# neverorfrog/vehicle-control

Hardware: AMD Instinct MI355X
Metric: MPC solves/sec (batched, N=20) (higher is better)
Workload: dtype f64; 1 GPU; C2 kinematic-bicycle LTV-MPC, B=1024 per GPU, N=20, fp64; batch_per_gpu=1024, global_batch=1024, horizon=20, parallelism=dp1 (independent shards)

## Files before the change

### include/vcmpc.h

```cpp
#ifndef VCMPC_H
#define VCMPC_H

#include <stdint.h>

#ifdef __cplusplus
extern "C" {
#endif

#define VCMPC_ABI_VERSION 13
#define VC_MAX_OBSTACLES 16

typedef struct vc_ctx vc_ctx;

enum vc_model { VC_MODEL_KINEMATIC = 0, VC_MODEL_DYNAMIC = 1, VC_MODEL_CASCADED = 2 };
enum vc_dtype { VC_F64 = 0, VC_F32 = 1 };
enum vc_flags { VC_HOST_PTRS = 0, VC_DEVICE_PTRS = 1 };
enum vc_tyre { VC_TYRE_FIALA = 0, VC_TYRE_LINEAR = 1 };
enum vc_status { VC_SOLVED = 0, VC_MAX_ITER = 1, VC_NONFINITE = 2, VC_OUT_OF_DOMAIN = 3, VC_INFEASIBLE = 4 };
enum vc_error {
  VC_OK = 0,
  VC_E_ARG = -1,
  VC_E_HIP = -2,
  VC_E_UNSUPPORTED = -3
};
// ... 71 lines not shown
int vc_abi_version(void);
int vc_params_sizeof(void);

vc_ctx* vc_create(int device, int model, int N, int max_batch, int dtype, const vc_params* params);
void vc_destroy(vc_ctx* ctx);
const char* vc_last_error(const vc_ctx* ctx);

int vc_set_stream(vc_ctx* ctx, void* stream);

int vc_set_obstacles(vc_ctx* ctx, int n, const double* s, const double* ey, const double* radius,
                     double margin_min);
int vc_synchronize(vc_ctx* ctx);

int vc_set_infeasibility(vc_ctx* ctx, int on, double eps);

int vc_get_farkas(vc_ctx* ctx, int B, void* y, int flags);

int vc_set_sqp_infeasibility(vc_ctx* ctx, int on, double eps);

int vc_get_sqp_farkas(vc_ctx* ctx, int B, void* y, int32_t* qp_index, int flags);

int vc_set_sqp_regularization(vc_ctx* ctx, int levels, double factor);

int vc_get_sqp_regularization(vc_ctx* ctx, int B, int32_t* level, int flags);

int vc_set_casc_infeasibility(vc_ctx* ctx, int on, double eps);

int vc_get_casc_farkas(vc_ctx* ctx, int B, void* y, int32_t* qp_index, int flags);

int vc_solve(vc_ctx* ctx, int B, const void* x0, const void* kappa, const void* ds,
             void* xbar, void* ubar, void* u0, int32_t* status, int32_t* iters, int flags);

int vc_solve_from(vc_ctx* ctx, int B, const void* x0, const void* kappa, const void* ds, const void* ubar_in,
                  void* xbar, void* u_out, void* u0, int32_t* status, int32_t* iters, int flags);

int vc_solve_diag(vc_ctx* ctx, int B, const void* x0, const void* kappa, const void* ds,
                  void* xbar, void* ubar, void* u0, int32_t* status, int32_t* iters, void* diag,
                  int flags);

int vc_solve_debug(vc_ctx* ctx, int B, const void* x0, const void* kappa, const void* ds, void* xbar, void* ubar,
                   void* u0, int32_t* status, int32_t* iters, void* dbg, int flags);
int vc_debug_stride(void);

int vc_debug_qp_fault(vc_ctx* ctx, int sqp_iter, int problem);

int vc_debug_kin_merit(vc_ctx* ctx, int B, const void* x0, const void* kappa, const void* ds, const void* u_prev,
                       void* u, const void* x_prev, void* x, int32_t* status, int32_t* iters, int32_t* st_acc,
                       int32_t* it_acc, int first, int restart, void* u0, void* ls_diag, int flags);

int vc_debug_sqp_breakdown(vc_ctx* ctx, int sqp_iter, int problem, int levels);

int vc_debug_rcp(vc_ctx* ctx, int n, const void* x, void* out, int flags);

int vc_rollout(vc_ctx* ctx, int B, const void* x0, const void* ubar, const void* kappa,
               const void* ds, void* xbar, int flags);

int vc_linearize(vc_ctx* ctx, int B, const void* xbar, const void* ubar, const void* kappa,
                 const void* ds, void* A, void* Bm, int flags);

int vc_condense(vc_ctx* ctx, int B, const void* x0, const void* ubar, const void* kappa,
                const void* ds, void* H, void* g, int flags);

int vc_plant_step(vc_ctx* ctx, int B, const void* x, const void* u, const void* kappa,
                  double dt, void* x_next, int flags);

int vc_spatial_step(vc_ctx* ctx, int B, const void* x, const void* u, const void* kappa,
                    const void* ds, void* x_next, int flags);

int vc_ode(vc_ctx* ctx, int B, const void* x, const void* u, const void* kappa, int space, void* f, int flags);

int vc_track_set(vc_ctx* ctx, int n_pieces, double h, double length, const double* coef);

int vc_track_k(vc_ctx* ctx, int B, const void* s, void* k, int flags);

int vc_horizon(vc_ctx* ctx, int B, const void* x0, const void* xbar, double mpc_dt, void* kappa, void* ds,
               int flags);

int vc_drive(vc_ctx* ctx, int B, double* x64, const void* u0, double dt, void* x_ctx, int flags);

int vc_simulate(vc_ctx* ctx, int B, int steps, double mpc_dt, double dt, double* x64, void* xbar, void* ubar,
                double* log_x, void* log_u, int32_t* nfail, int flags);

#ifdef __cplusplus
}
#endif
#endif
```

### vehicle-control_amd/csrc/kin_ltv.hip

```cpp
#include <hip/hip_runtime.h>

#include <cstdint>

#include "vc_kernels.hpp"
#include "vc_models.hpp"
#include "vcmpc.h"

#ifndef KIN_NU_TOL
#define KIN_NU_TOL 1e-10
#endif
#ifndef KIN_EARLY_F
#define KIN_EARLY_F 100.0
#endif
#ifndef KIN_EARLY_ROUNDS
#define KIN_EARLY_ROUNDS 2
#endif
#ifndef KIN_TAPIA_F
#define KIN_TAPIA_F 1.02
#endif
#ifndef KIN_DUAL_TOL
#define KIN_DUAL_TOL 1e-12
#endif
#ifndef KIN_AL_RHO
#define KIN_AL_RHO 1e1
// ... 136 lines not shown
  alignas(16) double zrow[48];
  double xb[N + 1][KIN_NX + 1];
  double jac[N + 1][9];
  double ub[D::n];
  double kap[N], ds[N];
  union {
    struct {
      double vz[64];
      double vc[64];
    };
    alignas(16) double tb2[128];
  };
  double dinv[64];
#if KIN_XPOSE_ONCE
  alignas(16) double tb3[8 * 18];
#endif
};
static_assert(sizeof(Smem<20>) <= 40960, "LDS of one problem: four must fit a CU's 160 KB");

template <int N>
__host__ __device__ constexpr int crow_stage(int r) {
  return r < N - 1 ? r + 1 : r - (N - 1) + 1;
}

template <int LEN, int SA, int SB, int CH = KIN_DOT_CH>
__device__ __forceinline__ double lds_dot(lds_cdouble* a, lds_cdouble* b) {
  constexpr int NCH = (LEN + CH - 1) / CH;
  double ca[2][CH], cb[2][CH];
  auto fetch = [&](int c, int buf) {
#pragma unroll
    for (int q = 0; q < CH; ++q) {
      const int i = c * CH + q;
      ca[buf][q] = (i < LEN) ? a[i * SA] : 0.0;
      cb[buf][q] = (i < LEN) ? b[i * SB] : 0.0;
    }
  };
  double a0 = 0.0, a1 = 0.0;
  fetch(0, 0);
#pragma unroll
  for (int c = 0; c < NCH; ++c) {
    if (c + 1 < NCH) fetch(c + 1, (c + 1) & 1);
    fence();
#pragma unroll
    for (int q = 0; q < CH; q += 2) {
      a0 += ca[c & 1][q] * cb[c & 1][q];
      a1 += ca[c & 1][q + 1] * cb[c & 1][q + 1];
    }
  }
  fence();
  return a0 + a1;
}

template <int N>
__device__ double grow_dot(const Smem<N>& s, int lane) {
  constexpr int NC = Dims<N>::NC;
  const int r = lane < NC ? lane : 0;
  const double a = lds_dot<2 * (N - 1), 1, 1>(lds_opaque(&s.G[r][0]), lds_opaque(&s.vz[0]));
  return lane < NC ? a : 0.0;
}

template <int N>
__device__ double gt_dot(const Smem<N>& s, int lane) {
  constexpr int n = Dims<N>::n, NC = Dims<N>::NC, LD = Dims<N>::LD;
  const int j = lane < n ? lane : 0;
  const double a = lds_dot<NC, LD, 1>(lds_opaque(&s.G[0][j]), lds_opaque(&s.vc[0]));
  return lane < n ? a : 0.0;
}


template <int N>
__device__ double h_dot(const Smem<N>& s, int lane) {
  constexpr int n = Dims<N>::n;
  const int j = lane < n ? lane : 0;
  return lds_dot<n, 1, 1>(lds_opaque(&s.H[j][0]), lds_opaque(&s.vz[0]));
}

__device__ __forceinline__ void kin_sincos(double x, double& sn, double& cs) {
  const double n = __builtin_rint(x * 6.36619772367581382433e-01);
  const double y = fma(-n, 6.07710050650619224932e-11, fma(-n, 1.57079632673412561417e+00, x));
  const double z = y * y;
  const double rs = fma(z, fma(z, fma(z, fma(z, 1.58969099521155010221e-10, -2.50507602534068634195e-08),
                                      2.75573137070700676789e-06), -1.98412698298579493134e-04),
                        8.33333333332248946124e-03);
  const double sk = fma(z * y, fma(z, rs, -1.66666666666666324348e-01), y);
  const double rc = z * fma(z, fma(z, fma(z, fma(z, fma(z, -1.13596475577881948265e-11, 2.08757232129817482790e-09),
                                                  -2.75573143513906633035e-07), 2.48015872894767294178e-05),
                                   -1.38888888888741095749e-03), 4.16666666666666019037e-02);
  const double hz = 0.5 * z, w = 1.0 - hz;
  const double ck = w + (((1.0 - w) - hz) + z * rc);
  const int q = int(n) & 3;
  const double a = (q & 1) ? ck : sk, b = (q & 1) ? sk : ck;
  sn = (q & 2) ? -a : a;
  cs = ((q + 1) & 2) ? -b : b;
}

__device__ __forceinline__ double rsq_nr(double d) {
  double inv = __builtin_amdgcn_rsq(d);
#if KIN_RSQ_HALLEY
  const double e = fma(-d, inv * inv, 1.0);
  return fma(inv * e, fma(0.375, e, 0.5), inv);
#else
  inv = inv * (1.5 - 0.5 * d * inv * inv);
  inv = inv * (1.5 - 0.5 * d * inv * inv);
  return inv;
#endif
}

template <int N>
__device__ __forceinline__ void store_rows(const double (&Mr)[Dims<N>::n], Smem<N>& s, int lane) {
}

template <int N>
struct RowRegs {
  int lo[Dims<N>::n], hi[Dims<N>::n];
};
template <int N>
__device__ __forceinline__ void row_put(RowRegs<N>& R, int k, double v) {
  asm("v_accvgpr_write_b32 %0, %1" : "=a"(R.lo[k]) : "v"(__double2loint(v)));
  asm("v_accvgpr_write_b32 %0, %1" : "=a"(R.hi[k]) : "v"(__double2hiint(v)));
// ... 682 lines not shown
    bx.hasLo = bx.hasHi = (lane < n);
    const int st = crow_stage<N>(lane < NC ? lane : 0);
    if (lane < N - 1) {
      cs.lo = W.v_min - s.xb[st][0];
      cs.hi = 0.0;
      cs.hasLo = true; cs.hasHi = false;
    } else if (lane < NC) {
      cs.lo = W.delta_min - s.xb[st][1];
      cs.hi = W.delta_max - s.xb[st][1];
      cs.hasLo = cs.hasHi = true;
    } else {
      cs.lo = cs.hi = 0.0;
      cs.hasLo = cs.hasHi = false;
    }
  }
  const double mtot = double(4 * N + 3 * (N - 1));
  double scale, hdiag_max;
  {
    double m = fabs(gj);
    if (bx.hasLo) m = fmax(m, fabs(bx.lo));
    if (bx.hasHi) m = fmax(m, fabs(bx.hi));
    if (cs.hasLo) m = fmax(m, fabs(cs.lo));
    if (cs.hasHi) m = fmax(m, fabs(cs.hi));
    scale = 1.0 + wave_max(m);
    hdiag_max = fmax(wave_max(hjj), 1.0);
  }
  double z = 0.0;
  bx.slo = bx.hasLo ? fmax(-bx.lo, 1.0) : 1.0;
  bx.shi = bx.hasHi ? fmax(bx.hi, 1.0) : 1.0;
  bx.llo = bx.hasLo ? 1.0 : 0.0;
  bx.lhi = bx.hasHi ? 1.0 : 0.0;
  cs.slo = cs.hasLo ? fmax(-cs.lo, 1.0) : 1.0;
  cs.shi = cs.hasHi ? fmax(cs.hi, 1.0) : 1.0;
  cs.llo = cs.hasLo ? 1.0 : 0.0;
  cs.lhi = cs.hasHi ? 1.0 : 0.0;

  VC_TACC(T_SETUP, t_setup0)
  const int max_iter = A.qp.max_iter;
  const double tol = A.qp.tol * scale;
  int it = 0;
  bool converged = false, chol_fail = false, near = false;
  double last_res = 0.0, last_mu = 0.0;
  RowRegs<N> Mr;
  double rd = 0.0, rlo_b = 0.0, rhi_b = 0.0, rlo_c = 0.0, rhi_c = 0.0;
  auto true_residuals = [&]() {
    wave_sync();
    s.vz[lane] = (lane < n) ? z : 0.0;
    s.vc[lane] = (lane < NC) ? (cs.lhi - cs.llo) : 0.0;
    wave_sync();
    const double yc = grow_dot<N>(s, lane);
    fence();
    const double hz = h_dot<N>(s, lane);
    fence();
    rd = (lane < n) ? (hz + gj + (bx.lhi - bx.llo) + gt_dot<N>(s, lane)) : 0.0;
    rlo_b = bx.hasLo ? (z - bx.lo - bx.slo) : 0.0;
    rhi_b = bx.hasHi ? (bx.hi - z - bx.shi) : 0.0;
    rlo_c = cs.hasLo ? (yc - cs.lo - cs.slo) : 0.0;
    rhi_c = cs.hasHi ? (cs.hi - yc - cs.shi) : 0.0;
  };
  auto max_residual = [&]() {
    return wave_max(fmax(fmax(fabs(rd), fmax(fabs(rlo_b), fabs(rhi_b))), fmax(fabs(rlo_c), fabs(rhi_c))));
  };
  int tapb = 0;
  const double tol_early = KIN_EARLY_F > 0.0 ? fmax(tol, KIN_EARLY_F * tol) : tol;
  int e_set = 0;
#ifdef VC_TIMING
  uint64_t e_fmask = 0;
  bool e_row = false, e_have = false;
#endif
  double tol_cur = tol_early;
  bool polished = false, pchol_fail = false;
  int rounds = 0;
#pragma unroll 1
  for (;;) {
  if (finite) {
#pragma unroll 1
    for (;;) {
      no_hoist();
      VC_TSTAMP(t_res0)
      if (it == 0) true_residuals();
      const double mu = wave_sum(__builtin_fma(cs.shi, cs.lhi,
                                               __builtin_fma(cs.slo, cs.llo,
                                                             __builtin_fma(bx.shi, bx.lhi, bx.slo * bx.llo)))) / mtot;
      double res = max_residual();
      if (it > 0 && res <= tol_cur && mu <= tol_cur) {
        true_residuals();
        res = max_residual();
      }
      converged = res <= tol_cur && mu <= tol_cur;
      last_res = res;
      last_mu = mu;
      if (converged || it >= max_iter || !isfinite(res) || !isfinite(mu)) break;
      ++it;
      const double wlo_b = bx.hasLo ? bx.llo / bx.slo : 0.0;
      const double whi_b = bx.hasHi ? bx.lhi / bx.shi : 0.0;
      const double wlo_c = cs.hasLo ? cs.llo / cs.slo : 0.0;
      const double whi_c = cs.hasHi ? cs.lhi / cs.shi : 0.0;
      wave_sync();
      s.vc[lane] = (lane < NC) ? wlo_c + whi_c : 0.0;
      wave_sync();
      VC_TACC(T_RESID, t_res0)
      VC_TSTAMP(t_build0)
      d4 nacc[Tiles<N>::NT];
      build_normal_acc<N>(nacc, s, wlo_b + whi_b, hjj, lane);
      VC_TACC(T_BUILD, t_build0)
      VC_TSTAMP(t_chol0)
      const bool chol_ok = factor_blocked<N>(Mr, nacc, s, lane);
      VC_TACC(T_CHOL, t_chol0)
      if (!chol_ok) {
        chol_fail = true;
        near = res <= 1e-6 * scale && mu <= tol;
        break;
      }
#ifdef VC_TIMING
      const uint64_t t_sol_before = tacc[T_SOLVE];
#endif
      VC_TSTAMP(t_step0)
      const double islo_b = bx.hasLo ? rcp_nr(bx.slo) : 0.0, ishi_b = bx.hasHi ? rcp_nr(bx.shi) : 0.0;
      const double islo_c = cs.hasLo ? rcp_nr(cs.slo) : 0.0, ishi_c = cs.hasHi ? rcp_nr(cs.shi) : 0.0;
      const double illo_b = bx.hasLo ? rcp_nr(bx.llo) : 0.0, ilhi_b = bx.hasHi ? rcp_nr(bx.lhi) : 0.0;
      const double illo_c = cs.hasLo ? rcp_nr(cs.llo) : 0.0, ilhi_c = cs.hasHi ? rcp_nr(cs.lhi) : 0.0;
      double sm = 0.0, pp1 = 0.0, pp2 = 0.0, pp3 = 0.0, pp4 = 0.0;
#pragma unroll 1
      for (int pass = 0; pass < 2; ++pass) {
        no_hoist();
        const double rclo_b = __builtin_fma(bx.slo, bx.llo, pp1) - sm, rchi_b = __builtin_fma(bx.shi, bx.lhi, pp2) - sm;
        const double rclo_c = __builtin_fma(cs.slo, cs.llo, pp3) - sm, rchi_c = __builtin_fma(cs.shi, cs.lhi, pp4) - sm;
        const double thi_b = ishi_b * -rchi_b, thi_c = ishi_c * -rchi_c;
        const double tlo_b = islo_b * rclo_b, tlo_c = islo_c * rclo_c;
        const double eb = (bx.hasHi ? __builtin_fma(-whi_b, rhi_b, thi_b) : 0.0) +
                          (bx.hasLo ? __builtin_fma(wlo_b, rlo_b, tlo_b) : 0.0);
        const double ec = (cs.hasHi ? __builtin_fma(-whi_c, rhi_c, thi_c) : 0.0) +
                          (cs.hasLo ? __builtin_fma(wlo_c, rlo_c, tlo_c) : 0.0);
        wave_sync();
        s.vc[lane] = (lane < NC) ? ec : 0.0;
        wave_sync();
        const double rhs = (lane < n) ? (-rd - eb - gt_dot<N>(s, lane)) : 0.0;
        VC_TSTAMP(t_sol0)
        const double dz = chol_solve<N>(Mr, s, rhs, lane);
        VC_TACC(T_SOLVE, t_sol0)
        wave_sync();
        s.vz[lane] = (lane < n) ? dz : 0.0;
        wave_sync();
        const double dyc = grow_dot<N>(s, lane);
        const double d1 = bx.hasLo ? dz + rlo_b : 0.0;
        const double d2 = bx.hasLo ? __builtin_fma(islo_b, -rclo_b, -(wlo_b * (dz + rlo_b))) : 0.0;
        const double d3 = bx.hasHi ? rhi_b - dz : 0.0;
        const double d4 = bx.hasHi ? __builtin_fma(-whi_b, rhi_b - dz, thi_b) : 0.0;
        const double e1 = cs.hasLo ? dyc + rlo_c : 0.0;
        const double e2 = cs.hasLo ? __builtin_fma(islo_c, -rclo_c, -(wlo_c * (dyc + rlo_c))) : 0.0;
        const double e3 = cs.hasHi ? rhi_c - dyc : 0.0;
        const double e4 = cs.hasHi ? __builtin_fma(-whi_c, rhi_c - dyc, thi_c) : 0.0;
        const double tmax = wave_max(fmax(fmax(fmax(-d1 * islo_b, -d2 * illo_b), fmax(-d3 * ishi_b, -d4 * ilhi_b)),
                                          fmax(fmax(-e1 * islo_c, -e2 * illo_c), fmax(-e3 * ishi_c, -e4 * ilhi_c))));
        const double amax = 1.0 / fmax(1.0, tmax);
        if (pass == 0) {
          const double mua = wave_sum((bx.slo + amax * d1) * (bx.llo + amax * d2) +
                                      (bx.shi + amax * d3) * (bx.lhi + amax * d4) +
                                      (cs.slo + amax * e1) * (cs.llo + amax * e2) +
                                      (cs.shi + amax * e3) * (cs.lhi + amax * e4)) / mtot;
          const double sr = mua / mu;
          sm = sr * sr * sr * mu;
          pp1 = d1 * d2; pp2 = d3 * d4; pp3 = e1 * e2; pp4 = e3 * e4;
        } else {
          const double al = KIN_STEP_F * amax;
          {
            auto tap = [&](double dl, double il, double dsv, double is) -> int {
              const double lr = fma(al * dl, il, 1.0), sr = fma(al * dsv, is, 1.0);
              return lr > KIN_TAPIA_F * sr ? 1 : (sr > KIN_TAPIA_F * lr ? 2 : 0);
            };
            tapb = tap(d2, illo_b, d1, islo_b) | (tap(d4, ilhi_b, d3, ishi_b) << 2) |
                   (tap(e2, illo_c, e1, islo_c) << 4) | (tap(e4, ilhi_c, e3, ishi_c) << 6);
          }
          z = (lane < n) ? z + al * dz : z;
          bx.slo += al * d1; bx.llo += al * d2; bx.shi += al * d3; bx.lhi += al * d4;
          cs.slo += al * e1; cs.llo += al * e2; cs.shi += al * e3; cs.lhi += al * e4;
          const double om = 1.0 - al;
          rd *= om; rlo_b *= om; rhi_b *= om; rlo_c *= om; rhi_c *= om;
        }
      }
      VC_TACC(T_STEP, t_step0)
#ifdef VC_TIMING
      tacc[T_STEP] -= tacc[T_SOLVE] - t_sol_before;
#endif
    }
  }

  VC_TSTAMP(t_pol0)
  if ((converged || near) && A.qp.polish > 0) {
    constexpr double AL_RHO = KIN_AL_RHO;
// ... 47 lines not shown
      const double rho_new = (act && gn2 > 1e-28) ? AL_RHO * hdiag_max / gn2 : 0.0;
      const double rho_c = (KIN_UPDATE && rho_k > 0.0 && rho_new > 0.0) ? rho_k : rho_new;
      const double bnd_c = act ? ((alo_c ? cs.lo : cs.hi) - gfix) : 0.0;
      const double base = (lane < n) ? -(gj + h_dot<N>(s, lane)) : 0.0;
      wave_sync();
      s.vc[lane] = rho_c;
      wave_sync();
      VC_TSTAMP(t_pf0)
      bool updated = false;
      if (KIN_UPDATE && upd != 0) {
        const bool same = __ballot(lane < NC && rho_c != rho_k && !(upd == 2 && lane == upd_j)) == 0ull;
        VC_TSTAMP(t_u0)
        if (same) updated = factor_update<N>(Mr, s, upd, upd_j, fixed, sqrt(lane_bcast(rho_c, upd_j)), lane);
#ifdef VC_TIMING
        if (updated) tacc[T_NUPD] += 1;
#endif
        VC_TACC(T_UCYC, t_u0)
      }
      rho_k = rho_c;
      if (!updated) {
        d4 pacc[Tiles<N>::NT];
        build_normal_acc<N>(pacc, s, 0.0, hjj, lane);
        const int pl = lane_opaque(lane), plr = pl >> 4, plc = pl & 15;
#pragma unroll
        for (int I = 0, t = 0; I < Tiles<N>::NB; ++I) {
#pragma unroll
          for (int J = 0; J <= I; ++J, ++t) {
            const int c = 16 * J + plc;
            const bool fc = (fmask >> c) & 1ull;
#pragma unroll
            for (int q = 0; q < 4; ++q) {
              const int r = 16 * I + plr + 4 * q;
              const bool fr = (fmask >> r) & 1ull;
              pacc[t][q] = (fr || fc) ? (r == c ? 1.0 : 0.0) : pacc[t][q];
            }
          }
        }
        if (!factor_blocked<N>(Mr, pacc, s, lane)) {
          pchol_fail = true;
          break;
        }
      }
      VC_TACC(T_UPDATE, t_pf0)
      VC_TSTAMP(t_pal0)
      double nu_c = (act && rho_c > 0.0) ? ((ahi_c ? cs.lhi : 0.0) - (alo_c ? cs.llo : 0.0)) : 0.0;

      const bool al_act = act && rho_c > 0.0;
      const double bnd_al = alo_c ? cs.lo : cs.hi;
      double zp = 0.0, emax = 0.0;
      {
        wave_sync();
        s.vc[lane] = (lane < NC) ? (nu_c - rho_c * bnd_c) : 0.0;
        wave_sync();
        const double rhs = (lane < n) ? (fixed ? zfix : (base - gt_dot<N>(s, lane))) : 0.0;
        zp = chol_solve<N>(Mr, s, rhs, lane);
        wave_sync();
        s.vz[lane] = (lane < n) ? zp : 0.0;
        wave_sync();
        const double yr = grow_dot<N>(s, lane);
        double rr = al_act ? (yr - bnd_al) : 0.0;
        const double ie = 1.0 / (1e-14 * scale), inu = KIN_NU_TOL > 0.0 ? 1.0 / (KIN_NU_TOL * scale) : 0.0;
        auto crit = [&](double r) { return wave_max(fmax(fabs(r) * ie, fabs(rho_c * r) * inu)); };
#ifdef VC_TIMING
        tacc[T_PPASS] += 1;
#endif
        if (crit(rr) > 1.0) {
          double pd = rho_c * rr;
          double rz = wave_sum(rr * pd);
#pragma unroll 1
          for (int it = 1; it < AL_MAX; ++it) {
            no_hoist();
            wave_sync();
            s.vc[lane] = (lane < NC) ? pd : 0.0;
            wave_sync();
            const double gtp = gt_dot<N>(s, lane);
            const double zq = chol_solve<N>(Mr, s, (lane < n && !fixed) ? gtp : 0.0, lane);
            wave_sync();
            s.vz[lane] = (lane < n) ? zq : 0.0;
            wave_sync();
            const double gq = grow_dot<N>(s, lane);
            const double q = al_act ? gq : 0.0;
            const double pq = wave_sum(pd * q);
#ifdef VC_TIMING
            tacc[T_PPASS] += 1;
#endif
            if (!(pq > 0.0)) break;
            const double al = rz / pq;
            nu_c = fma(al, pd, nu_c);
            zp = fma(-al, zq, zp);
            rr = fma(-al, q, rr);
            if (crit(rr) <= 1.0) break;
            const double zt = rho_c * rr;
            const double rzn = wave_sum(rr * zt);
            pd = fma(rzn / rz, pd, zt);
            rz = rzn;
          }
        }
      }
      VC_TACC(T_PAL, t_pal0)
      wave_sync();
      s.vz[lane] = (lane < n) ? zp : 0.0;
      s.vc[lane] = (lane < NC) ? nu_c : 0.0;
      wave_sync();
      const double grad = (lane < n) ? (h_dot<N>(s, lane) + gj + gt_dot<N>(s, lane)) : 0.0;
      const double ypc = grow_dot<N>(s, lane);
#if KIN_STAT_CHECK
      emax = wave_max(fmax(al_act ? fabs(ypc - bnd_al) : 0.0, (lane < n && !fixed) ? fabs(grad) : 0.0));
#else
      emax = wave_max(al_act ? fabs(ypc - bnd_al) : 0.0);
#endif
      const double dv_b = (lane < n) ? (ahi_b ? grad : (alo_b ? -grad : -1.0)) : -1.0;
      const double dv_c = (lane < NC) ? (ahi_c ? -nu_c : (alo_c ? nu_c : -1.0)) : -1.0;
      const double pv_b = (lane < n && !fixed) ? fmax(bx.lo - zp, zp - bx.hi) : -1.0;
      const double pv_c = (lane < NC && !(act && rho_c > 0.0))
                              ? fmax(cs.hasLo ? cs.lo - ypc : -1.0, cs.hasHi ? ypc - cs.hi : -1.0)
                              : -1.0;
      const double dmax = wave_max(fmax(dv_b, dv_c));
      const double pmax = wave_max(fmax(pv_b, pv_c));
      if (dmax <= dtol && pmax <= ptol) {
        if (emax <= ptol) {
          z = (lane < n) ? zp : z;
          polished = true;
        }
        break;
      }
      const bool dual = dmax > dtol;
      const double worst = dual ? dmax : pmax;
      const double vb = dual ? dv_b : pv_b, vcr = dual ? dv_c : pv_c;
      const uint64_t who = __ballot(fmax(vb, vcr) == worst);
      const int sel = __builtin_ffsll((long long)who) - 1;
      const bool sel_box = (__ballot(vb >= vcr) >> sel) & 1ull;
      upd = dual ? 0 : (sel_box ? 1 : 2);
      upd_j = sel;
#ifdef VC_TIMING
      if (dual) tacc[T_NDROP] += 1;
#endif
      if (lane == sel) {
        if (vb >= vcr) {
          if (dual) { alo_b = false; ahi_b = false; }
          else if (zp < bx.lo) alo_b = true;
          else ahi_b = true;
        } else {
          if (dual) { alo_c = false; ahi_c = false; }
          else if (ypc < cs.lo) alo_c = true;
          else ahi_c = true;
        }
      }
#ifdef VC_TIMING
      int r0code = 0;
      if (tol_cur > tol && round == 0) {
        int tside = 0;
        if (vb >= vcr) tside = (dual ? (ahi_b ? (tapb >> 2) : tapb) : (zp < bx.lo ? tapb : (tapb >> 2))) & 3;
        else tside = (dual ? (ahi_c ? (tapb >> 6) : (tapb >> 4)) : (ypc < cs.lo ? (tapb >> 4) : (tapb >> 6))) & 3;
        const int code = 1 + (dual ? 2 : (vb >= vcr ? 0 : 1)) + 3 * tside;
        r0code = __builtin_amdgcn_readlane(code, sel);
#ifdef VC_TIMING
        tacc[T_R0CHG] = (uint64_t)r0code;
// ... 48 lines not shown
  }
  {
    const double y = grow_dot<N>(s, lane);
    const int slot = lane < N - 1 ? 64 + lane + 1
                                  : (lane < NC ? n + (lane - (N - 1)) + 1 : (lane == NC ? 64 : (lane == NC + 1 ? n : 127)));
    wave_sync();
    s.tb2[slot] = y;
    wave_sync();
    double ey = 0.0, ep = 0.0, eyk = 0.0, epk = 0.0;
#pragma unroll 4
    for (int k = 0; k < N; ++k) {
      const double h = s.ds[k], dd = s.vz[n + k];
      eyk = lane_put(eyk, ey, k);
      epk = lane_put(epk, ep, k);
      const double ney = ey + h * (s.jac[k][4] * ey + s.jac[k][5] * ep);
      const double nep = ep + h * (s.jac[k][6] * dd + s.jac[k][7] * ey + s.jac[k][8] * ep);
      ey = ney; ep = nep;
    }
    eyk = lane_put(eyk, ey, N);
    epk = lane_put(epk, ep, N);
    const double eyn = __shfl_down(eyk, 1), epn = __shfl_down(epk, 1);
    const int k = lane < N ? lane : 0;
    const double q = s.jac[k][0], qv = s.jac[k][1], qey = s.jac[k][2], qep = s.jac[k][3];
    const double h = s.ds[k], a = s.ub[2 * k], w = s.ub[2 * k + 1];
    const double da = s.vz[2 * k], dw = s.vz[2 * k + 1];
    const double dv = s.vc[k], dd = s.vz[n + k];
    const double dq = qv * dv + qey * eyk + qep * epk;
    const double dt = wave_prefix(lane < N ? h * dq : 0.0, lane);
    wave_sync();
    if (lane < N) {
      double* xr = s.xb[k + 1];
      xr[0] += dv + h * (a * dq + q * da);
      xr[1] += dd + h * (w * dq + q * dw);
      xr[3] += eyn;
      xr[4] += epn;
      xr[5] += dt;
    }
    wave_sync();
    double* xo = A.x_out + (size_t)b * (N + 1) * KIN_NX;
    for (int i = lane; i < (N + 1) * KIN_NX; i += 64) xo[i] = s.xb[i / KIN_NX][i % KIN_NX];
  }
  VC_TACC(T_OUT, t_out0)
  VC_TACC(T_TOTAL, t_all0)
#ifdef VC_TIMING
  if (A.diag && lane < T_NSLOT) {
    double v = 0.0;
#pragma unroll
    for (int i = 0; i < T_NSLOT; ++i) v = (i == lane) ? double(tacc[i]) : v;
    A.diag[(size_t)b * (4 + T_NSLOT) + 4 + lane] = v;
  }
#endif
}

size_t kin_ltv_smem_bytes(int N) {
  switch (N) {
    case 20: return sizeof(Smem<20>);
    default: return 0;
  }
}

hipError_t launch_kin_ltv(const KinLtvArgs& a, int N, hipStream_t stream) {
  if (a.B <= 0) return hipSuccess;
  switch (N) {
    case 20:
      hipLaunchKernelGGL(kin_ltv_kernel<20>, dim3(a.B), dim3(64), 0, stream, a);
      return hipGetLastError();
    default:
      return hipErrorInvalidValue;
  }
}

}
```

### vehicle-control_amd/csrc/vc_kernels.hpp

```cpp
#pragma once
#include <hip/hip_runtime.h>

#include <cstddef>
#include <cstdint>

#include "vc_models.hpp"
#include "vcmpc.h"

#ifdef VC_TIMING
#define VC_DIAG_COLS 16
#define VC_DYN_DIAG_COLS 19
#define VC_CASC_DIAG_COLS 17
#define VC_ST_DIAG_COLS 13
#else
#define VC_DIAG_COLS 4
#define VC_DYN_DIAG_COLS 4
#define VC_CASC_DIAG_COLS 4
#define VC_ST_DIAG_COLS 4
#endif

#define VC_OBS_MARGIN_MIN 0.05

namespace vc {

// ... 198 lines not shown
  double* u0;
  int32_t* status;
  int32_t* iters;
  double* diag;
  double* jws;
  double* H_out;
  double* g_out;
  int mode;
  int B;
  DynCoef<double> car;
  vc_dyn_mpc w;
  vc_casc_mpc cw;
  vc_qp qp;
  vc_obstacles obs;
  int detect;
  double detect_eps;
  double* farkas;
  int32_t* qp_index;
};

struct ModelArgs {
  int model;
  int B, N;
  int M;
  int shift;
  double L;
  DynCoef<double> dyn64;
  DynCoef<float> dyn32;
};
template <typename T>
__host__ __device__ inline const DynCoef<T>& dyn_coef(const ModelArgs& m);
template <>
__host__ __device__ inline const DynCoef<double>& dyn_coef<double>(const ModelArgs& m) { return m.dyn64; }
template <>
__host__ __device__ inline const DynCoef<float>& dyn_coef<float>(const ModelArgs& m) { return m.dyn32; }

struct TrackTable {
  const double* coef;
  int n;
  double h, length;
};

hipError_t launch_track_k(const TrackTable& tt, int dtype, int B, const void* s, void* k, hipStream_t st);
hipError_t launch_horizon(const TrackTable& tt, int model, int dtype, int B, int N, int M, double ds_pm,
                          const void* x0, bool x0_fp64, const void* xbar, double mpc_dt, void* kappa, void* ds,
                          void* x0_out, hipStream_t st);
hipError_t launch_drive(const ModelArgs& m, int dtype, const TrackTable& tt, double* x64, const void* u0, double dt,
                        void* x_ctx, const int32_t* status, void* xbar, void* ubar, int32_t* nfail, double* log_x,
                        void* log_u, const void* kappa, hipStream_t st);
hipError_t launch_kin_ltv(const KinLtvArgs& a, int N, hipStream_t stream);
hipError_t launch_kin_ric(const KinLtvArgs& a, int N, hipStream_t stream);
hipError_t launch_kin_merit(const KinMeritArgs& a, hipStream_t stream);
hipError_t launch_rcp_probe(int n, const double* x, double* out, hipStream_t st);
hipError_t launch_kin_qp_fault(const KinLtvArgs& a, int N, int b, hipStream_t stream);
bool kin_ric_built(int N);
hipError_t launch_dyn_sqp(const DynSqpArgs& a, int N, hipStream_t stream);
hipError_t launch_casc_sqp(const CascSqpArgs& a, int N, int M, hipStream_t stream);
hipError_t launch_casc_ric(const CascSqpArgs& a, int N, int M, hipStream_t stream);
bool casc_ric_built(int N, int M);
size_t casc_ric_jws_doubles(int N, int M, int B);
hipError_t launch_st_sqp(const StSqpArgs& a, int N, hipStream_t stream);
hipError_t launch_st_sqp_reg(const StSqpArgs& a, int N, hipStream_t stream);
bool st_sqp_built(int N);
size_t st_sqp_jws_doubles(int N, int B);
bool casc_sqp_built(int N, int M);
size_t dyn_sqp_smem_bytes(int N);
int dyn_sqp_debug_stride();
size_t kin_ltv_smem_bytes(int N);
hipError_t launch_ode(const ModelArgs& m, int dtype, const void* x, const void* u, const void* kappa, int space,
                      void* f, hipStream_t st);
hipError_t launch_plant_step(const ModelArgs& m, int dtype, const void* x, const void* u, const void* kappa, double dt,
                             void* xn, hipStream_t st);
hipError_t launch_spatial_step(const ModelArgs& m, int dtype, const void* x, const void* u, const void* kappa,
                               const void* ds, void* xn, hipStream_t st);
hipError_t launch_rollout(const ModelArgs& m, int dtype, const void* x0, const void* ubar, const void* kappa,
                          const void* ds, void* xbar, hipStream_t st);
hipError_t launch_kin_linearize(const ModelArgs& m, const void* xbar, const void* ubar, const void* kappa,
                                const void* ds, void* A, void* Bm, hipStream_t st);

}
```

### vehicle-control_amd/csrc/vcmpc_abi.hip

```cpp
#include <hip/hip_runtime.h>

#include <cmath>
#include <cstdarg>
#include <cstdio>
#include <cstring>
#include <string>
#include <vector>

#include "vc_kernels.hpp"
#include "vcmpc.h"


struct Detect {
  bool on = false;
  double eps = 1e-9;
  void* farkas = nullptr;
  void* qp_index = nullptr;
  size_t rows = 0;
  int B = 0;
};

struct Regularize {
  int levels = 0;
  double factor = 10.0;
// ... 669 lines not shown
    m.obs = a.obs;
    const bool elastic_retry = c->p.qp.elastic < 0.0 && !kin_condensed(c);
    if (c->p.qp.elastic < 0.0) a.qp.elastic = 0.0;
    for (int i = 0; i < S; ++i) {
      VC_HIP(c, hipMemcpyAsync(base + o_up, a.u_out, u_bytes, hipMemcpyDeviceToDevice, c->stream));
      if (m.ms) VC_HIP(c, hipMemcpyAsync(base + o_xp, a.x_out, x_bytes, hipMemcpyDeviceToDevice, c->stream));
      if (kin_condensed(c)) VC_HIP(c, vc::launch_kin_ltv(a, N, c->stream));
      else VC_HIP(c, vc::launch_kin_ric(a, N, c->stream));
      if (elastic_retry) {
        vc::KinLtvArgs e = a;
        e.qp.elastic = c->p.qp.elastic;
        e.ubar = (const double*)(base + o_up);
        if (m.ms) e.x_in = (const double*)(base + o_xp);
        VC_HIP(c, vc::launch_kin_ric(e, N, c->stream));
      }
      if (i == c->fault_iter && c->fault_problem >= 0 && c->fault_problem < B)
        VC_HIP(c, vc::launch_kin_qp_fault(a, N, c->fault_problem, c->stream));
      m.first = i == 0;
      VC_HIP(c, vc::launch_kin_merit(m, c->stream));
    }
  }
  return st.finish();
}

int vc_solve_debug(vc_ctx* c, int B, const void* x0, const void* kappa, const void* ds, void* xbar, void* ubar,
                   void* u0, int32_t* status, int32_t* iters, void* dbg, int flags) {
  if (int r = check_common(c, B, flags)) return r;
  if (!dyn_solve_built(c)) return fail(c, VC_E_UNSUPPORTED, "vc_solve_debug: dynamic fp32 N=40 contexts only");
  if (!x0 || !kappa || !ds || !xbar || !ubar || !u0 || !status || !iters || !dbg)
    return fail(c, VC_E_ARG, "null pointer");
  if (B == 0) return 0;
  return dyn_solve(c, B, x0, kappa, ds, xbar, ubar, u0, status, iters, nullptr, flags, dbg);
}

int vc_debug_stride(void) { return vc::dyn_sqp_debug_stride(); }

int vc_debug_rcp(vc_ctx* c, int n, const void* x, void* out, int flags) {
  if (!c) return VC_E_ARG;
  if (n < 0 || n > c->max_batch) return fail(c, VC_E_ARG, "n %d outside [0, max_batch=%d]", n, c->max_batch);
  if (int r = check_common(c, 0, flags)) return r;
  if (!x || !out) return fail(c, VC_E_ARG, "null pointer");
  if (n == 0) return 0;
  Ptr dx, dout;
  Staging st(c, flags);
  if (int r = st.bind([&] {
        dx = st.in(x, (size_t)n * 8);
        dout = st.out(out, (size_t)n * 32);
      }))
    return r;
  VC_HIP(c, vc::launch_rcp_probe(n, dx, dout, c->stream));
  return st.finish();
}

int vc_debug_qp_fault(vc_ctx* c, int sqp_iter, int problem) {
  if (!c) return VC_E_ARG;
  c->fault_iter = sqp_iter;
  c->fault_problem = problem;
  return 0;
}

int vc_debug_kin_merit(vc_ctx* c, int B, const void* x0, const void* kappa, const void* ds, const void* u_prev,
                       void* u, const void* x_prev, void* x, int32_t* status, int32_t* iters, int32_t* st_acc,
                       int32_t* it_acc, int first, int restart, void* u0, void* ls_diag, int flags) {
  if (int r = check_common(c, B, flags)) return r;
  if (c->model != VC_MODEL_KINEMATIC || c->dtype != VC_F64)
    return fail(c, VC_E_UNSUPPORTED, "vc_debug_kin_merit: kinematic fp64 contexts only; model=%d dtype=%d", c->model,
                c->dtype);
  const bool ms = c->p.qp.ms != 0;
  if (!x0 || !kappa || !ds || !u_prev || !u || !x || !status || !iters || !st_acc || !it_acc || !u0 || !ls_diag ||
      (ms && !x_prev))
    return fail(c, VC_E_ARG, "null pointer");
  if (B == 0) return 0;
  const int N = c->N, nx = 6, nu = 2;
  const size_t u_bytes = (size_t)B * N * nu * 8, x_bytes = (size_t)B * (N + 1) * nx * 8;
  vc::KinMeritArgs m{};
  m.B = B;
  m.N = N;
  m.first = first != 0;
  m.restart = restart != 0;
  m.ms = ms;
  m.L = c->p.kin_car.l;
  m.w = c->p.kin_mpc;
  m.obs = c->p.obs;
  Staging st(c, flags);
  if (int r = st.bind([&] {
        m.x0 = st.in(x0, (size_t)B * nx * 8);
        m.kappa = st.in(kappa, (size_t)B * N * 8);
        m.ds = st.in(ds, (size_t)B * N * 8);
        m.u_prev = st.in(u_prev, u_bytes);
        m.ubar = st.inout(u, u_bytes);
        m.x_out = st.pair(ms ? x : nullptr, x, x_bytes).wr;
        m.x_prev = ms ? (const double*)st.in(x_prev, x_bytes) : (const double*)m.x_out;
        m.qp_status = m.status = st.inout(status, (size_t)B * 4);
        m.qp_iters = m.iters = st.inout(iters, (size_t)B * 4);
        m.st_acc = st.inout(st_acc, (size_t)B * 4);
        m.it_acc = st.inout(it_acc, (size_t)B * 4);
        m.u0 = st.out(u0, (size_t)B * nu * 8);
        m.ls_diag = st.out(ls_diag, (size_t)B * 4 * 8);
      }))
    return r;
  VC_HIP(c, vc::launch_kin_merit(m, c->stream));
  return st.finish();
}

int vc_condense(vc_ctx* c, int B, const void* x0, const void* ubar, const void* kappa, const void* ds, void* H,
                void* g, int flags) {
// ... 271 lines not shown
```

### vehicle-control_amd/vcmpc/_abi.py

```python
from __future__ import annotations

import ctypes as C
import os

LIB_NAME = "libvcmpc.so"
LIB_PATH = os.environ.get("VCMPC_LIB", os.path.join(os.path.dirname(os.path.abspath(__file__)), LIB_NAME))
ABI_VERSION = 13
VC_MAX_OBSTACLES = 16
OBS_MARGIN_MIN = 0.05

VC_MODEL_KINEMATIC, VC_MODEL_DYNAMIC, VC_MODEL_CASCADED = 0, 1, 2
VC_F64, VC_F32 = 0, 1
VC_HOST_PTRS, VC_DEVICE_PTRS = 0, 1
VC_TYRE_FIALA, VC_TYRE_LINEAR = 0, 1
VC_SOLVED, VC_MAX_ITER, VC_NONFINITE, VC_OUT_OF_DOMAIN, VC_INFEASIBLE = 0, 1, 2, 3, 4
VC_OK, VC_E_ARG, VC_E_HIP, VC_E_UNSUPPORTED = 0, -1, -2, -3

STATUS_NAMES = {VC_SOLVED: "solved", VC_MAX_ITER: "max_iter", VC_NONFINITE: "nonfinite",
                VC_OUT_OF_DOMAIN: "out_of_domain", VC_INFEASIBLE: "infeasible"}


class vc_kin_car(C.Structure):
    _fields_ = [("l", C.c_double)]

# ... 27 lines not shown

class vc_obstacles(C.Structure):
    _fields_ = [("n", C.c_int32), ("inside", C.c_int32), ("margin_min", C.c_double),
                ("s", C.c_double * VC_MAX_OBSTACLES), ("ey", C.c_double * VC_MAX_OBSTACLES),
                ("radius", C.c_double * VC_MAX_OBSTACLES)]


class vc_casc_mpc(C.Structure):
    _fields_ = [("horizon_pm", C.c_int32), ("pad_", C.c_int32)] + [(k, C.c_double) for k in (
        "ds_pm", "w_dev_pm", "w_Fy", "w_switch", "V_min", "ey_min_pm", "ey_max_pm")]


class vc_params(C.Structure):
    _fields_ = [("kin_car", vc_kin_car), ("dyn_car", vc_dyn_car), ("kin_mpc", vc_kin_mpc), ("qp", vc_qp),
                ("dyn_mpc", vc_dyn_mpc), ("obs", vc_obstacles), ("casc", vc_casc_mpc)]


class VcError(RuntimeError):

    def __init__(self, code: int, msg: str):
        super().__init__(f"vcmpc error {code}: {msg}")
        self.code = code


_vp = C.c_void_p
_i32p = C.POINTER(C.c_int32)

PROTOTYPES = {
    "vc_abi_version": (C.c_int, []),
    "vc_params_sizeof": (C.c_int, []),
    "vc_create": (_vp, [C.c_int, C.c_int, C.c_int, C.c_int, C.c_int, C.POINTER(vc_params)]),
    "vc_destroy": (None, [_vp]),
    "vc_last_error": (C.c_char_p, [_vp]),
    "vc_set_stream": (C.c_int, [_vp, _vp]),
    "vc_synchronize": (C.c_int, [_vp]),
    "vc_set_obstacles": (C.c_int, [_vp, C.c_int, _vp, _vp, _vp, C.c_double]),
    "vc_set_infeasibility": (C.c_int, [_vp, C.c_int, C.c_double]),
    "vc_get_farkas": (C.c_int, [_vp, C.c_int, _vp, C.c_int]),
    "vc_set_sqp_infeasibility": (C.c_int, [_vp, C.c_int, C.c_double]),
    "vc_get_sqp_farkas": (C.c_int, [_vp, C.c_int, _vp, _vp, C.c_int]),
    "vc_set_sqp_regularization": (C.c_int, [_vp, C.c_int, C.c_double]),
    "vc_get_sqp_regularization": (C.c_int, [_vp, C.c_int, _vp, C.c_int]),
    "vc_debug_sqp_breakdown": (C.c_int, [_vp, C.c_int, C.c_int, C.c_int]),
    "vc_set_casc_infeasibility": (C.c_int, [_vp, C.c_int, C.c_double]),
    "vc_get_casc_farkas": (C.c_int, [_vp, C.c_int, _vp, _vp, C.c_int]),
    "vc_solve": (C.c_int, [_vp, C.c_int, _vp, _vp, _vp, _vp, _vp, _vp, _vp, _vp, C.c_int]),
    "vc_solve_diag": (C.c_int, [_vp, C.c_int, _vp, _vp, _vp, _vp, _vp, _vp, _vp, _vp, _vp, C.c_int]),
    "vc_solve_from": (C.c_int, [_vp, C.c_int, _vp, _vp, _vp, _vp, _vp, _vp, _vp, _vp, _vp, C.c_int]),
    "vc_solve_debug": (C.c_int, [_vp, C.c_int, _vp, _vp, _vp, _vp, _vp, _vp, _vp, _vp, _vp, C.c_int]),
    "vc_debug_stride": (C.c_int, []),
    "vc_debug_qp_fault": (C.c_int, [_vp, C.c_int, C.c_int]),
    "vc_debug_kin_merit": (C.c_int, [_vp, C.c_int] + [_vp] * 11 + [C.c_int, C.c_int, _vp, _vp, C.c_int]),
    "vc_debug_rcp": (C.c_int, [_vp, C.c_int, _vp, _vp, C.c_int]),
    "vc_rollout": (C.c_int, [_vp, C.c_int, _vp, _vp, _vp, _vp, _vp, C.c_int]),
    "vc_linearize": (C.c_int, [_vp, C.c_int, _vp, _vp, _vp, _vp, _vp, _vp, C.c_int]),
    "vc_condense": (C.c_int, [_vp, C.c_int, _vp, _vp, _vp, _vp, _vp, _vp, C.c_int]),
    "vc_plant_step": (C.c_int, [_vp, C.c_int, _vp, _vp, _vp, C.c_double, _vp, C.c_int]),
    "vc_spatial_step": (C.c_int, [_vp, C.c_int, _vp, _vp, _vp, _vp, _vp, C.c_int]),
    "vc_ode": (C.c_int, [_vp, C.c_int, _vp, _vp, _vp, C.c_int, _vp, C.c_int]),
    "vc_track_set": (C.c_int, [_vp, C.c_int, C.c_double, C.c_double, _vp]),
    "vc_track_k": (C.c_int, [_vp, C.c_int, _vp, _vp, C.c_int]),
    "vc_horizon": (C.c_int, [_vp, C.c_int, _vp, _vp, C.c_double, _vp, _vp, C.c_int]),
    "vc_drive": (C.c_int, [_vp, C.c_int, _vp, _vp, C.c_double, _vp, C.c_int]),
    "vc_simulate": (C.c_int, [_vp, C.c_int, C.c_int, C.c_double, C.c_double, _vp, _vp, _vp, _vp, _vp, _vp, C.c_int]),
}

_LIB = None


def load_library(path: str | None = None) -> C.CDLL:
    global _LIB
    if _LIB is not None and path is None:
        return _LIB
    p = path or LIB_PATH
    try:
        import torch
    except ImportError:
        pass
    if not os.path.exists(p):
        raise ImportError(
            f"{p} not found: build it with `make -C vehicle-control_amd/csrc` "
            "(or __graft_entry__.build()); vcmpc has no CPU fallback")
    lib = C.CDLL(p)
    for name, (res, args) in PROTOTYPES.items():
        fn = getattr(lib, name)
        fn.restype = res
        fn.argtypes = args
    if lib.vc_abi_version() != ABI_VERSION:
        raise ImportError(f"{p}: ABI version {lib.vc_abi_version()} != {ABI_VERSION}")
    if lib.vc_params_sizeof() != C.sizeof(vc_params):
        raise ImportError(f"{p}: sizeof(vc_params) {lib.vc_params_sizeof()} != ctypes {C.sizeof(vc_params)}")
    if path is None:
        _LIB = lib
    return lib


def check(lib, ctx, code: int) -> None:
    if code != VC_OK:
        msg = lib.vc_last_error(ctx)
        raise VcError(code, msg.decode() if msg else "")
```

Baseline: 5.548 million solves/s.

## Split G row/column dot products across idle wave lanes with bpermute reduction

Rewrites grow_dot and gt_dot so that the lanes which sat idle in the 64-wide wave (beyond NC or n) compute the second half of long rows and columns. The partial sums come back through ds_bpermute, and short rows keep their whole sum in a stash. The goal is to shorten the serial LDS-load and FMA chain inside the per-iteration QP loop. In exchange it adds lane-index arithmetic and a cross-lane exchange, and the lane plan is hard-coded for N=20. A debug kernel and ABI entry are also added to test the new dot products.

```diff
diff --git a/include/vcmpc.h b/include/vcmpc.h
--- a/include/vcmpc.h
+++ b/include/vcmpc.h
@@ -147,6 +147,9 @@
 
 int vc_debug_rcp(vc_ctx* ctx, int n, const void* x, void* out, int flags);
 
+int vc_debug_kin_gdots(vc_ctx* ctx, int B, const void* G, const void* vz, const void* vc, void* out_grow,
+                       void* out_gt, int flags);
+
 int vc_rollout(vc_ctx* ctx, int B, const void* x0, const void* ubar, const void* kappa,
                const void* ds, void* xbar, int flags);
 
diff --git a/vehicle-control_amd/csrc/kin_ltv.hip b/vehicle-control_amd/csrc/kin_ltv.hip
--- a/vehicle-control_amd/csrc/kin_ltv.hip
+++ b/vehicle-control_amd/csrc/kin_ltv.hip
@@ -212,19 +212,105 @@
 }
 
 template <int N>
+struct GSplit {
+  static_assert(N == 20, "the lane plan below is worked out for N = 20 (the one instantiation)");
+  static constexpr int NC = Dims<N>::NC, n = Dims<N>::n, LD = Dims<N>::LD;
+  static constexpr int T = NC / 2;
+  static constexpr int ROW_SHORT = T - (T + 1) / 2;
+  static_assert(NC + 2 * (N - 1 - ROW_SHORT) <= 64, "partner lanes of the long rows");
+  static constexpr int COL_LONG = n / 2;
+  static_assert(n + COL_LONG <= 64, "partner lanes of the long columns");
+};
+
+__device__ __forceinline__ double lane_fetch(double v, int byte_lane) {
+  const int lo = __builtin_amdgcn_ds_bpermute(byte_lane, __double2loint(v));
+  const int hi = __builtin_amdgcn_ds_bpermute(byte_lane, __double2hiint(v));
+  return __hiloint2double(hi, lo);
+}
+
+template <int T0, int T1, int GS, int D>
+__device__ __forceinline__ void gsplit_fetch(double (&a)[5], double (&b)[5], uint32_t g, uint32_t v) {
+  static_assert(2 * T0 - D >= 0, "offsets from a segment base are not negative");
+  lds_cdouble* gp = (lds_cdouble*)(uintptr_t)g;
+  lds_cdouble* vp = (lds_cdouble*)(uintptr_t)v;
+#pragma unroll
+  for (int t = T0; t < T1; ++t) {
+    a[t - T0] = gp[(2 * t - D) * GS];
+    b[t - T0] = vp[2 * t - D];
+  }
+}
+template <int CNT>
+__device__ __forceinline__ double gsplit_fma(const double (&a)[5], const double (&b)[5], double acc) {
+#pragma unroll
+  for (int q = 0; q < CNT; ++q) acc = __builtin_fma(a[q], b[q], acc);
+  return acc;
+}
+template <int N, int GS, int D2, int D3>
+__device__ __forceinline__ double gsplit_chain(const uint32_t (&g)[4], const uint32_t (&v)[4], bool shrt,
+                                               double& stash) {
+  static_assert(GSplit<N>::T == 19, "segments of 5, 5, 4 and 5 steps");
+  double a0[5], b0[5], a1[5], b1[5];
+  gsplit_fetch<0, 5, GS, 0>(a0, b0, g[0], v[0]);
+  gsplit_fetch<5, 10, GS, 0>(a1, b1, g[1], v[1]);
+  fence();
+  double acc = gsplit_fma<5>(a0, b0, 0.0);
+  gsplit_fetch<10, 14, GS, D2>(a0, b0, g[2], v[2]);
+  fence();
+  acc = gsplit_fma<5>(a1, b1, acc);
+  gsplit_fetch<14, 19, GS, D3>(a1, b1, g[3], v[3]);
+  fence();
+  stash = acc;
+  acc = shrt ? 0.0 : acc;
+  acc = gsplit_fma<4>(a0, b0, acc);
+  fence();
+  acc = gsplit_fma<5>(a1, b1, acc);
+  fence();
+  return acc;
+}
+
+template <int N>
 __device__ double grow_dot(const Smem<N>& s, int lane) {
-  constexpr int NC = Dims<N>::NC;
-  const int r = lane < NC ? lane : 0;
-  const double a = lds_dot<2 * (N - 1), 1, 1>(lds_opaque(&s.G[r][0]), lds_opaque(&s.vz[0]));
-  return lane < NC ? a : 0.0;
+  using P = GSplit<N>;
+  constexpr int NC = P::NC, LD = P::LD;
+  const int l = lane_opaque(lane);
+  const bool part = l >= NC;
+  const bool shrt = uint32_t(l) < uint32_t(P::ROW_SHORT) || uint32_t(l - (N - 1)) < uint32_t(P::ROW_SHORT);
+  const int r = min(part ? l - (l < NC + (N - 1 - P::ROW_SHORT) ? NC - P::ROW_SHORT : N) : l, NC);
+  const uint32_t odd = part ? 8u : 0u;
+  const uint32_t fwd = shrt ? 0u : 8u * uint32_t(P::T);
+  const uint32_t g0 = (uint32_t)(uintptr_t)(lds_cdouble*)&s.G[0][0] + uint32_t(r) * (8u * LD) + odd;
+  const uint32_t v0 = (uint32_t)(uintptr_t)(lds_cdouble*)&s.vz[0] + odd;
+  const uint32_t g[4] = {g0, g0, g0 + fwd, g0 + fwd}, v[4] = {v0, v0, v0 + fwd, v0 + fwd};
+  double stash;
+  const double acc = gsplit_chain<N, 1, P::T, P::T>(g, v, shrt, stash);
+  const double other = lane_fetch(acc, 4 * (l + (l < N - 1 ? NC - P::ROW_SHORT : N)));
+  const double y = acc + (shrt ? stash : other);
+  return l < NC ? y : 0.0;
 }
 
 template <int N>
 __device__ double gt_dot(const Smem<N>& s, int lane) {
-  constexpr int n = Dims<N>::n, NC = Dims<N>::NC, LD = Dims<N>::LD;
-  const int j = lane < n ? lane : 0;
-  const double a = lds_dot<NC, LD, 1>(lds_opaque(&s.G[0][j]), lds_opaque(&s.vc[0]));
-  return lane < n ? a : 0.0;
+  using P = GSplit<N>;
+  constexpr int n = P::n, LD = P::LD;
+  const int l = lane_opaque(lane);
+  const bool part = l >= n;
+  const bool shrt = uint32_t(l - P::COL_LONG) < uint32_t(n - P::COL_LONG);
+  const int j = part ? l - n : l;
+  const uint32_t ms = shrt ? 1u : 0u, mp = part ? 1u : 0u;
+  const uint32_t gp = (uint32_t)(uintptr_t)(lds_cdouble*)&s.G[0][0] + uint32_t(j) * 8u + mp * (8u * LD);
+  const uint32_t vp = (uint32_t)(uintptr_t)(lds_cdouble*)&s.vc[0] + mp * 8u;
+  constexpr int SH[4] = {10, 18, 0, 1}, D[4] = {0, 0, 9, 0};
+  uint32_t g[4], v[4];
+#pragma unroll
+  for (int k = 0; k < 4; ++k) {
+    g[k] = gp + uint32_t(D[k] * 8 * LD) + ms * uint32_t((SH[k] - D[k]) * 8 * LD);
+    v[k] = vp + uint32_t(D[k] * 8) + ms * uint32_t((SH[k] - D[k]) * 8);
+  }
+  double stash;
+  const double acc = gsplit_chain<N, LD, D[2], D[3]>(g, v, shrt, stash);
+  const double other = lane_fetch(acc, 4 * (l + n));
+  const double y = acc + (shrt ? stash : other);
+  return l < n ? y : 0.0;
 }
 
 
@@ -1013,7 +1099,8 @@
     fence();
     const double hz = h_dot<N>(s, lane);
     fence();
-    rd = (lane < n) ? (hz + gj + (bx.lhi - bx.llo) + gt_dot<N>(s, lane)) : 0.0;
+    const double gtl = gt_dot<N>(s, lane);
+    rd = (lane < n) ? (hz + gj + (bx.lhi - bx.llo) + gtl) : 0.0;
     rlo_b = bx.hasLo ? (z - bx.lo - bx.slo) : 0.0;
     rhi_b = bx.hasHi ? (bx.hi - z - bx.shi) : 0.0;
     rlo_c = cs.hasLo ? (yc - cs.lo - cs.slo) : 0.0;
@@ -1096,7 +1183,8 @@
         wave_sync();
         s.vc[lane] = (lane < NC) ? ec : 0.0;
         wave_sync();
-        const double rhs = (lane < n) ? (-rd - eb - gt_dot<N>(s, lane)) : 0.0;
+        const double gte = gt_dot<N>(s, lane);
+        const double rhs = (lane < n) ? (-rd - eb - gte) : 0.0;
         VC_TSTAMP(t_sol0)
         const double dz = chol_solve<N>(Mr, s, rhs, lane);
         VC_TACC(T_SOLVE, t_sol0)
@@ -1250,7 +1338,8 @@
         wave_sync();
         s.vc[lane] = (lane < NC) ? (nu_c - rho_c * bnd_c) : 0.0;
         wave_sync();
-        const double rhs = (lane < n) ? (fixed ? zfix : (base - gt_dot<N>(s, lane))) : 0.0;
+        const double gtn = gt_dot<N>(s, lane);
+        const double rhs = (lane < n) ? (fixed ? zfix : (base - gtn)) : 0.0;
         zp = chol_solve<N>(Mr, s, rhs, lane);
         wave_sync();
         s.vz[lane] = (lane < n) ? zp : 0.0;
@@ -1300,7 +1389,8 @@
       s.vz[lane] = (lane < n) ? zp : 0.0;
       s.vc[lane] = (lane < NC) ? nu_c : 0.0;
       wave_sync();
-      const double grad = (lane < n) ? (h_dot<N>(s, lane) + gj + gt_dot<N>(s, lane)) : 0.0;
+      const double gtnu = gt_dot<N>(s, lane);
+      const double grad = (lane < n) ? (h_dot<N>(s, lane) + gj + gtnu) : 0.0;
       const double ypc = grow_dot<N>(s, lane);
 #if KIN_STAT_CHECK
       emax = wave_max(fmax(al_act ? fabs(ypc - bnd_al) : 0.0, (lane < n && !fixed) ? fabs(grad) : 0.0));
@@ -1455,6 +1545,32 @@
 #endif
 }
 
+template <int N>
+__global__ __launch_bounds__(64) void kin_gdots_kernel(int B, const double* G, const double* vz, const double* vc,
+                                                       double* out_grow, double* out_gt) {
+  constexpr int n = Dims<N>::n, NC = Dims<N>::NC, LD = Dims<N>::LD;
+  __shared__ Smem<N> s;
+  const int lane = threadIdx.x;
+  const int b = blockIdx.x;
+  if (b >= B) return;
+  for (int i = lane; i < (NC + 3) * LD; i += 64) (&s.G[0][0])[i] = 0.0;
+  wave_sync();
+  for (int i = lane; i < NC * n; i += 64) s.G[i / n][i % n] = G[(size_t)b * NC * n + i];
+  s.vz[lane] = lane < n ? vz[(size_t)b * n + lane] : 0.0;
+  s.vc[lane] = lane < NC ? vc[(size_t)b * NC + lane] : 0.0;
+  wave_sync();
+  out_grow[(size_t)b * 64 + lane] = grow_dot<N>(s, lane);
+  out_gt[(size_t)b * 64 + lane] = gt_dot<N>(s, lane);
+}
+
+hipError_t launch_kin_gdots(int B, int N, const double* G, const double* vz, const double* vc, double* out_grow,
+                            double* out_gt, hipStream_t stream) {
+  if (B <= 0) return hipSuccess;
+  if (N != 20) return hipErrorInvalidValue;
+  hipLaunchKernelGGL(kin_gdots_kernel<20>, dim3(B), dim3(64), 0, stream, B, G, vz, vc, out_grow, out_gt);
+  return hipGetLastError();
+}
+
 size_t kin_ltv_smem_bytes(int N) {
   switch (N) {
     case 20: return sizeof(Smem<20>);
diff --git a/vehicle-control_amd/csrc/vc_kernels.hpp b/vehicle-control_amd/csrc/vc_kernels.hpp
--- a/vehicle-control_amd/csrc/vc_kernels.hpp
+++ b/vehicle-control_amd/csrc/vc_kernels.hpp
@@ -274,6 +274,8 @@
 hipError_t launch_kin_ric(const KinLtvArgs& a, int N, hipStream_t stream);
 hipError_t launch_kin_merit(const KinMeritArgs& a, hipStream_t stream);
 hipError_t launch_rcp_probe(int n, const double* x, double* out, hipStream_t st);
+hipError_t launch_kin_gdots(int B, int N, const double* G, const double* vz, const double* vc, double* out_grow,
+                            double* out_gt, hipStream_t stream);
 hipError_t launch_kin_qp_fault(const KinLtvArgs& a, int N, int b, hipStream_t stream);
 bool kin_ric_built(int N);
 hipError_t launch_dyn_sqp(const DynSqpArgs& a, int N, hipStream_t stream);
diff --git a/vehicle-control_amd/csrc/vcmpc_abi.hip b/vehicle-control_amd/csrc/vcmpc_abi.hip
--- a/vehicle-control_amd/csrc/vcmpc_abi.hip
+++ b/vehicle-control_amd/csrc/vcmpc_abi.hip
@@ -745,6 +745,28 @@
   return st.finish();
 }
 
+int vc_debug_kin_gdots(vc_ctx* c, int B, const void* G, const void* vz, const void* vc, void* out_grow,
+                       void* out_gt, int flags) {
+  if (int r = check_common(c, B, flags)) return r;
+  if (c->model != VC_MODEL_KINEMATIC || c->dtype != VC_F64 || vc::kin_ltv_smem_bytes(c->N) == 0)
+    return fail(c, VC_E_UNSUPPORTED, "vc_debug_kin_gdots: kinematic fp64 contexts with the fused kernel's N only");
+  if (!G || !vz || !vc || !out_grow || !out_gt) return fail(c, VC_E_ARG, "null pointer");
+  if (B == 0) return 0;
+  const int N = c->N, n = 2 * N, NC = 2 * (N - 1);
+  Ptr dG, dvz, dvc, dgrow, dgt;
+  Staging st(c, flags);
+  if (int r = st.bind([&] {
+        dG = st.in(G, (size_t)B * NC * n * 8);
+        dvz = st.in(vz, (size_t)B * n * 8);
+        dvc = st.in(vc, (size_t)B * NC * 8);
+        dgrow = st.out(out_grow, (size_t)B * 64 * 8);
+        dgt = st.out(out_gt, (size_t)B * 64 * 8);
+      }))
+    return r;
+  VC_HIP(c, vc::launch_kin_gdots(B, N, dG, dvz, dvc, dgrow, dgt, c->stream));
+  return st.finish();
+}
+
 int vc_debug_qp_fault(vc_ctx* c, int sqp_iter, int problem) {
   if (!c) return VC_E_ARG;
   c->fault_iter = sqp_iter;
diff --git a/vehicle-control_amd/vcmpc/_abi.py b/vehicle-control_amd/vcmpc/_abi.py
--- a/vehicle-control_amd/vcmpc/_abi.py
+++ b/vehicle-control_amd/vcmpc/_abi.py
@@ -103,6 +103,7 @@
     "vc_debug_qp_fault": (C.c_int, [_vp, C.c_int, C.c_int]),
     "vc_debug_kin_merit": (C.c_int, [_vp, C.c_int] + [_vp] * 11 + [C.c_int, C.c_int, _vp, _vp, C.c_int]),
     "vc_debug_rcp": (C.c_int, [_vp, C.c_int, _vp, _vp, C.c_int]),
+    "vc_debug_kin_gdots": (C.c_int, [_vp, C.c_int, _vp, _vp, _vp, _vp, _vp, C.c_int]),
     "vc_rollout": (C.c_int, [_vp, C.c_int, _vp, _vp, _vp, _vp, _vp, C.c_int]),
     "vc_linearize": (C.c_int, [_vp, C.c_int, _vp, _vp, _vp, _vp, _vp, _vp, C.c_int]),
     "vc_condense": (C.c_int, [_vp, C.c_int, _vp, _vp, _vp, _vp, _vp, _vp, C.c_int]),
```

Result: faster. 5.963 million solves/s, median of 6 (+7.5%).
